# Biblbrox/ViT-Spectre-Experiments

Measured on AMD Instinct MI355X. Metric: images/sec training, Spectre-ViT-S CIFAR-100 bs512, higher is better.
Workload: dtype bf16; 1 GPU; Spectre-ViT-Small (E512 H16 F768 L4 P4 N65, 100 classes, dropout 0.001), fft mixer, train step fwd+CE+bwd+AdamW, bs 512/GPU; mixer=fft, global_batch=512, parallelism=dp1

## Files before the change

include/spv.h:

```cpp
#ifndef SPV_H
#define SPV_H

#include <stddef.h>
#include <stdint.h>

#ifdef __cplusplus
extern "C" {
#endif

#define SPV_F32 0
#define SPV_BF16 1

#define SPV_ABI_VERSION 1

int spv_version(void);
enum {
    SPV_PATH_GEMM_STRIP = 0,
    SPV_PATH_GEMM_STRIP_ACC = 1,
    SPV_PATH_GEMM_TN = 2,
    SPV_PATH_TAIL_LC = 3,
    SPV_PATH_TAIL_UP = 4,
    SPV_PATH_TAIL_LN = 5,
    SPV_PATH_FNET_MFMA = 6,
    SPV_PATH_GATHER_LDS = 7,
// ... 212 lines not shown
#define SPV_HADAMARD_REFUSE_TOKENS (-4)
#define SPV_HADAMARD_REFUSE_WORKSPACE (-5)
int spv_hadamard_path(int dtype, int tokens, int dim, int has_workspace);
int64_t spv_hadamard_workspace_floats(int batch, int tokens, int dim);
int spv_hadamard_mix(const void* x, void* y, const void* add_in, int batch, int tokens, int dim, float scale, int dtype,
                     float* workspace, void* stream);
int spv_hadamard_ln_supported(int tokens, int dim, int dtype);
int spv_hadamard_ln_fwd(const void* x, void* prenorm, void* out, const float* gamma, const float* beta, float* mean, float* rstd,
                        float scale, int batch, int tokens, int dim, int dtype, void* stream);
int spv_hadamard_ln_bwd(const void* dout, const void* prenorm, const float* mean, const float* rstd, const float* gamma, void* dx,
                        float* dgamma, float* dbeta, float* partials, float scale, int batch, int tokens, int dim, int dtype,
                        void* stream);
int spv_hadamard_cls_supported(int tokens, int dim, int dtype);
int spv_hadamard_cls_fwd(const void* x, const float* gamma, const float* beta, void* out, float* m0, float* mean, float* rstd,
                         float scale, int batch, int tokens, int dim, int dtype, void* stream);
int spv_hadamard_cls_bwd(const void* g1, const float* m0, const float* mean, const float* rstd, const float* gamma, void* dx,
                         float* partials, float scale, int batch, int tokens, int dim, int dtype, void* stream);

int spv_patchify(const float* img, void* out, int batch, int chans, int height, int width, int patch, int ld,
                 int transposed, int out_dtype, void* stream);
int spv_patchify_u8(const unsigned char* img_hwc, const float* mean, const float* inv_std, void* out, int batch, int chans,
                    int height, int width, int patch, int ld, int transposed, int out_dtype, void* stream);
int spv_embed_posbias(const float* pos, const float* bias, const float* cls, float* out, int patches, int embed, void* stream);
int spv_embed_cls_rows(const float* cls, const float* pos, void* tokens, int batch, int tokens_per_image, int embed,
                       int dtype, void* stream);
int spv_spectral_fold(const float* proj_w, const float* freq_h, const float* freq_w, float* w_full, int embed,
                      int chans, int patch, void* stream);
int spv_spectral_fold_bf16(const float* proj_w, const float* freq_h, const float* freq_w, float* w_full, void* w_full_bf16, int embed,
                           int chans, int patch, void* stream);
int spv_spectral_fold_bwd(const float* dw_full, const float* proj_w, const float* freq_h, const float* freq_w,
                          float* dproj_w, float* dfreq_h, float* dfreq_w, float* scratch, int embed, int chans,
                          int patch, void* stream);
int spv_dropout(const void* x, void* y, int64_t n, float p, uint64_t seed, int dtype, void* stream);
int spv_embed_bwd_groups(int batch);
int spv_embed_bwd(const void* g, const void* gcls, void* dtok, float* partials, float* dpos, float* dbias, float* dcls, int batch,
                  int tokens, int embed, float p_drop, uint64_t seed, int dtype, void* stream);

int spv_attention_fwd(const void* qkv, void* ctx, void* probs, int seqs, int len, int heads, int head_dim, int dtype,
                      float p_drop, uint64_t seed, void* stream);
int spv_attention_bwd(const void* dctx, const void* qkv, const void* probs, void* dscores, void* dqkv, int seqs, int len,
                      int heads, int head_dim, int dtype, float p_drop, uint64_t seed, void* stream);
int spv_attention_row0_fwd(const void* q0, const void* k, const void* v, int ldkv, void* ctx0, float* probs, int batch, int len,
                           int heads, int head_dim, int dtype, float p_drop, uint64_t seed, void* stream);
int spv_attention_row0_bwd(const void* dctx0, const void* q0, const void* k, const void* v, int ldkv, const float* probs, void* dq0,
                           void* dk, void* dv, int ldd, int batch, int len, int heads, int head_dim, int dtype, float p_drop,
                           uint64_t seed, void* stream);

int spv_gelu_fwd(const void* x, void* y, int64_t n, int dtype, void* stream);
int spv_gelu_bwd(const void* dy, const void* x, void* dx, int64_t n, int dtype, void* stream);
int spv_colsum(const void* x, float* out, float* partials, int rows, int n, int dtype, void* stream);
int spv_axpby(const void* x, const void* y, void* out, float a, float b, int64_t n, int dtype, void* stream);

int spv_small_sl_supported(int rows, int n, int k);
int64_t spv_small_sl_partial_floats(int rows, int n);
int spv_small_sl_fwd(const void* xa, int64_t lda, const void* xb, int64_t ldb, const float* W, const float* bias,
                     const float* gamma, const float* beta, float* out, float* h, float* xs, float* mean, float* rstd,
                     int rows, int n, int k, int dtype, void* stream);
int spv_small_sl_bwd(const float* dout, const float* h, const float* xs, const float* mean, const float* rstd,
                     const float* W, const float* gamma, const float* beta, float* dh, void* dx, float* dW,
                     float* dgamma, float* dbeta, float* dbias, float* partials, int rows, int n, int k, int dx_dtype,
                     void* stream);
int spv_small_sl_bwd_rows(const float* dout, const float* h, const float* mean, const float* rstd, const float* W,
                          const float* gamma, const float* beta, float* dh, void* dx, float* partials, int rows, int n, int k,
                          int dx_dtype, void* stream);
int spv_small_sl_bwd_w(const float* dh, const float* xs, const float* partials, float* dW, float* dgamma, float* dbeta,
                       float* dbias, int rows, int n, int k, void* stream);
// ... 112 lines not shown
```

vit-spectre-experiments_amd/csrc/spv_patch.hip:

```cpp
#define SPV_USES_SEED
#include "spv_common.h"
#include "spv_prologue_core.h"

namespace {

__device__ __forceinline__ float ld_any(const void* base, size_t off, int bf) {
    return bf ? bf2f(static_cast<const bf16_t*>(base)[off]) : static_cast<const float*>(base)[off];
}

__global__ __launch_bounds__(256) void patchify_kernel(const float* __restrict__ img, void* __restrict__ out, int B, int C, int H,
                                                       int W, int P, int ld, int transposed, int bf) {
    patchify_body(img, out, B, C, H, W, P, ld, transposed, bf, blockIdx.x, gridDim.x);
}

template <typename T>
__global__ __launch_bounds__(256) void patchify_vec4_kernel(const float* __restrict__ img, T* __restrict__ out, int B, int C, int H, int W,
                                                            int P, int ld, int token_rows) {
    patchify_vec4_body<T>(img, out, B, C, H, W, P, ld, token_rows, blockIdx.x, gridDim.x);
}

__global__ __launch_bounds__(256) void patchify_u8_kernel(const unsigned char* __restrict__ img, const float* __restrict__ mean,
                                                          const float* __restrict__ inv_std, void* __restrict__ out, int B, int C,
                                                          int H, int W, int P, int ld, int transposed, int bf) {
    const int nH = H / P, nW = W / P, Np = nH * nW, K = C * P * P;
    const int64_t rows = (int64_t)B * Np;
    const int64_t total = transposed == 1 ? (int64_t)K * ld : (transposed == 2 ? (int64_t)B * (Np + 1) * ld : rows * ld);
    for (int64_t e = (int64_t)blockIdx.x * blockDim.x + threadIdx.x; e < total; e += (int64_t)gridDim.x * blockDim.x) {
        int64_t row;
        int k;
        if (transposed == 1) { k = (int)(e / ld); row = e % ld; }
        else { row = e / ld; k = (int)(e % ld); }
        if (transposed == 2) {
            const int64_t b2 = row / (Np + 1);
            const int t2 = (int)(row % (Np + 1));
            row = t2 == 0 ? rows : b2 * Np + t2 - 1;
// ... 77 lines not shown
    }
}
__global__ __launch_bounds__(1024) void freq_weight_grad_kernel(const float* __restrict__ gw, const float* __restrict__ fh,
                                                                const float* __restrict__ fw, float* __restrict__ dfh,
                                                                float* __restrict__ dfw, int EC, int P) {
    extern __shared__ float lds[];
    const int Pv = P / 2 + 1, S = P + Pv;
    const int nt = blockDim.x;
    float* mine = lds + threadIdx.x * S;
    for (int j = 0; j < S; ++j) mine[j] = 0.0f;
    for (int ec = threadIdx.x; ec < EC; ec += nt) {
        const float* g = gw + (size_t)ec * P * Pv;
        for (int u = 0; u < P; ++u)
            for (int v = 0; v < Pv; ++v) {
                const float t = g[u * Pv + v];
                mine[u] += t * fw[v];
                mine[P + v] += t * fh[u];
            }
    }
    for (int stride = nt >> 1; stride >= 1; stride >>= 1) {
        __syncthreads();
        if ((int)threadIdx.x < stride) {
            const float* other = lds + (threadIdx.x + stride) * S;
            for (int j = 0; j < S; ++j) mine[j] += other[j];
        }
    }
    if (threadIdx.x == 0) {
        for (int j = 0; j < P; ++j) dfh[j] = mine[j];
        for (int j = 0; j < Pv; ++j) dfw[j] = mine[P + j];
    }
}

inline int ew_blocks(int64_t n) { return patch_ew_blocks(n); }

}

extern "C" int spv_patchify(const float* img, void* out, int batch, int chans, int height, int width, int patch, int ld,
                            int transposed, int out_dtype, void* stream) {
    SPV_CHECK(batch > 0 && chans > 0 && patch > 0 && height >= patch && width >= patch, "spv_patchify: bad shape");
    SPV_CHECK(out_dtype == SPV_F32 || out_dtype == SPV_BF16, "spv_patchify: bad dtype");
    const int Np = (height / patch) * (width / patch), K = chans * patch * patch;
    const int64_t rows = (int64_t)batch * Np;
    SPV_CHECK(transposed >= 0 && transposed <= 2 && (transposed == 1 ? ld >= rows : ld >= K), "spv_patchify: ld=%d too small", ld);
    const int64_t total = transposed == 1 ? (int64_t)K * ld : (transposed == 2 ? (int64_t)batch * (Np + 1) * ld : rows * ld);
    if (transposed != 1 && patch % 4 == 0 && width % 4 == 0 && ld % 4 == 0 && ((uintptr_t)img & 15) == 0 && ((uintptr_t)out & 15) == 0) {
        const int64_t vecs = (int64_t)batch * (Np + (transposed == 2 ? 1 : 0)) * (ld / 4);
        if (out_dtype == SPV_BF16)
            hipLaunchKernelGGL((patchify_vec4_kernel<bf16_t>), dim3(ew_blocks(vecs)), dim3(256), 0, static_cast<hipStream_t>(stream), img, (bf16_t*)out,
                               batch, chans, height, width, patch, ld, transposed == 2);
        else
            hipLaunchKernelGGL((patchify_vec4_kernel<float>), dim3(ew_blocks(vecs)), dim3(256), 0, static_cast<hipStream_t>(stream), img, (float*)out,
                               batch, chans, height, width, patch, ld, transposed == 2);
        SPV_LAUNCH_CHECK("spv_patchify(vec4)");
        return 0;
    }
    hipLaunchKernelGGL(patchify_kernel, dim3(ew_blocks(total)), dim3(256), 0, static_cast<hipStream_t>(stream), img, out, batch,
                       chans, height, width, patch, ld, transposed, out_dtype == SPV_BF16);
    SPV_LAUNCH_CHECK("spv_patchify");
    return 0;
}

extern "C" int spv_patchify_u8(const unsigned char* img_hwc, const float* mean, const float* inv_std, void* out, int batch,
                               int chans, int height, int width, int patch, int ld, int transposed, int out_dtype, void* stream) {
    SPV_CHECK(batch > 0 && chans > 0 && patch > 0 && height >= patch && width >= patch, "spv_patchify_u8: bad shape");
    SPV_CHECK(out_dtype == SPV_F32 || out_dtype == SPV_BF16, "spv_patchify_u8: bad dtype");
    SPV_CHECK(mean != nullptr && inv_std != nullptr, "spv_patchify_u8: mean / inv_std missing");
    const int Np = (height / patch) * (width / patch), K = chans * patch * patch;
    const int64_t rows = (int64_t)batch * Np;
    SPV_CHECK(transposed >= 0 && transposed <= 2 && (transposed == 1 ? ld >= rows : ld >= K), "spv_patchify_u8: ld=%d too small", ld);
    const int64_t total = transposed == 1 ? (int64_t)K * ld : (transposed == 2 ? (int64_t)batch * (Np + 1) * ld : rows * ld);
    hipLaunchKernelGGL(patchify_u8_kernel, dim3(ew_blocks(total)), dim3(256), 0, static_cast<hipStream_t>(stream), img_hwc, mean,
                       inv_std, out, batch, chans, height, width, patch, ld, transposed, out_dtype == SPV_BF16);
    SPV_LAUNCH_CHECK("spv_patchify_u8");
    return 0;
}

extern "C" int spv_embed_posbias(const float* pos, const float* bias, const float* cls, float* out, int patches, int embed, void* stream) {
    SPV_CHECK(patches > 0 && embed > 0, "spv_embed_posbias: empty");
    hipLaunchKernelGGL(posbias_kernel, dim3(ew_blocks((int64_t)(patches + 1) * embed)), dim3(256), 0, static_cast<hipStream_t>(stream), pos,
                       bias, cls, out, patches, embed);
    SPV_LAUNCH_CHECK("spv_embed_posbias");
    return 0;
}

extern "C" int spv_embed_cls_rows(const float* cls, const float* pos, void* tokens, int batch, int tokens_per_image, int embed,
                                  int dtype, void* stream) {
    SPV_CHECK(batch > 0 && tokens_per_image > 0 && embed > 0, "spv_embed_cls_rows: empty");
    SPV_CHECK(dtype == SPV_F32 || dtype == SPV_BF16, "spv_embed_cls_rows: bad dtype");
    hipLaunchKernelGGL(cls_rows_kernel, dim3(ew_blocks((int64_t)batch * embed)), dim3(256), 0, static_cast<hipStream_t>(stream), cls,
                       pos, tokens, batch, tokens_per_image, embed, dtype == SPV_BF16);
    SPV_LAUNCH_CHECK("spv_embed_cls_rows");
    return 0;
}

constexpr int EB_GS = 16, EB_HB = 8;
template <typename T>
__global__ __launch_bounds__(256) void embed_bwd_rows_kernel(const T* __restrict__ g, const T* __restrict__ gcls, T* __restrict__ dtok,
                                                            float* __restrict__ partials, int B, int TE, int E, float p, uint64_t seed) {
    const int v = blockIdx.x * 256 + threadIdx.x;
    if (v * 8 >= TE) return;
    const int col = v * 8;
    const int b0 = blockIdx.y * EB_GS;
    const float inv_keep = 1.0f / (1.0f - p);
    const uint64_t sd = live_seed(seed);
    float acc[8];
#pragma unroll
    for (int u = 0; u < 8; ++u) acc[u] = 0.0f;
    const bool cls_row = gcls != nullptr && col < E;
    if constexpr (sizeof(T) == 2) {
        typedef unsigned raw4 __attribute__((ext_vector_type(4)));
        for (int h0 = 0; h0 < EB_GS; h0 += EB_HB) {
            raw4 xr[EB_HB], cr[EB_HB];
#pragma unroll
            for (int s = 0; s < EB_HB; ++s) xr[s] = *reinterpret_cast<const raw4*>(g + (size_t)min(b0 + h0 + s, B - 1) * TE + col);
            if (cls_row) {
#pragma unroll
                for (int s = 0; s < EB_HB; ++s) cr[s] = *reinterpret_cast<const raw4*>(gcls + (size_t)min(b0 + h0 + s, B - 1) * E + col);
            }
#pragma unroll
            for (int s = 0; s < EB_HB; ++s) {
                const int b = b0 + h0 + s;
                if (b >= B) break;
                const size_t i = (size_t)b * TE + col;
                float x[8];
// ... 182 lines not shown
```

vit-spectre-experiments_amd/spectre_vit/_native.py:

```python
import ctypes
import os

import torch

_HERE = os.path.dirname(os.path.abspath(__file__))
LIB_PATH = os.environ.get("SPV_LIB_PATH") or os.path.join(os.path.dirname(_HERE), "lib", "libspv_hip.so")

c_vp, c_i, c_i64, c_u64, c_f, c_d = ctypes.c_void_p, ctypes.c_int, ctypes.c_int64, ctypes.c_uint64, ctypes.c_float, ctypes.c_double

PATH = dict(gemm_strip=0, gemm_strip_acc=1, gemm_tn=2, tail_lc=3, tail_up=4, tail_ln=5, fnet_mfma=6, gather_lds=7, distill_cached=8, gemm_tn_wide=9,
            gemm_tn_batch=10, gemm_strip_pool=11, permut_row0=12, gemm_rows=13,
            spectrum=14, conv_fwd=15, conv_dgrad=16, conv_wgrad=17, token_pool=18, token_unpool=19, attn_row0_fwd=20, attn_row0_bwd=21, augment=22, teacher_view=23,
            attn_v1=24, attn_v2=25, attn_v3=26)

SIGNATURES = {
    "spv_version": [],
    "spv_last_error": [],
    "spv_path_count": [c_i],
    "spv_cast": [c_vp, c_i, c_vp, c_i, c_i64, c_vp],
    "spv_cast_transpose": [c_vp, c_i, c_vp, c_i, c_i, c_i, c_i, c_i, c_i, c_i, c_vp],
    "spv_weight_shadows": [c_vp, c_vp, c_vp, c_i, c_i, c_i, c_i, c_vp],
    "spv_weight_shadows_multi": [c_vp, c_vp, c_vp, c_vp, c_i, c_i, c_vp],
    "spv_gemm_nt": [c_vp, c_vp, c_vp, c_vp, c_i, c_i, c_i, c_i, c_i, c_i, c_i, c_i, c_i, c_i, c_vp, c_vp],
    "spv_gemm_nt_grouped_rows": [c_vp, c_vp, c_vp, c_vp, c_vp, c_i, c_i, c_i, c_i, c_i, c_i, c_i, c_i, c_i, c_i, c_i, c_vp],
# ... 29 lines not shown
    "spv_gemm_tn_batch_part": [c_vp, c_i, c_i, c_i, c_vp, c_vp, c_i, c_i, c_vp],
    "spv_small_sl_supported": [c_i, c_i, c_i],
    "spv_small_sl_partial_floats": [c_i, c_i],
    "spv_small_sl_fwd": [c_vp, c_i64, c_vp, c_i64, c_vp, c_vp, c_vp, c_vp, c_vp, c_vp, c_vp, c_vp, c_vp, c_i, c_i, c_i, c_i, c_vp],
    "spv_small_sl_bwd": [c_vp] * 15 + [c_i, c_i, c_i, c_i, c_vp],
    "spv_small_sl_bwd_rows": [c_vp] * 10 + [c_i, c_i, c_i, c_i, c_vp],
    "spv_small_sl_bwd_w": [c_vp] * 7 + [c_i, c_i, c_i, c_vp],
    "spv_cross_entropy_workspace_floats": [],
    "spv_cross_entropy_fwd": [c_vp, c_vp, c_vp, c_vp, c_vp, c_i, c_i, c_vp],
    "spv_cross_entropy_bwd": [c_vp, c_vp, c_vp, c_vp, c_vp, c_i, c_i, c_vp],
    "spv_permut_gather_fwd": [c_vp, c_vp, c_vp, c_vp, c_i, c_i, c_i, c_i, c_i, c_vp],
    "spv_gemm_nt_pool_bwd": [c_vp, c_vp, c_vp, c_vp, c_i, c_i, c_i, c_i, c_i, c_i, c_i, c_i, c_i, c_i, c_vp],
    "spv_permut_gather_bwd": [c_vp, c_vp, c_vp, c_i, c_i, c_i, c_i, c_vp],
    "spv_fnet_mix": [c_vp, c_vp, c_vp, c_vp, c_i, c_i, c_i, c_i, c_vp, c_vp],
    "spv_fnet_workspace_floats": [c_i, c_i, c_i],
    "spv_fnet_twiddle_floats": [c_i],
    "spv_fnet_make_twiddle": [c_vp, c_i, c_vp],
    "spv_fnet_ln_supported": [c_i, c_i, c_i],
    "spv_fnet_cls_supported": [c_i, c_i, c_i],
    "spv_fnet_cls_fwd": [c_vp, c_vp, c_vp, c_vp, c_vp, c_vp, c_vp, c_i, c_i, c_i, c_i, c_vp],
    "spv_fnet_cls_bwd": [c_vp, c_vp, c_vp, c_vp, c_vp, c_vp, c_vp, c_i, c_i, c_i, c_i, c_vp],
    "spv_fnet_ln_fwd": [c_vp, c_vp, c_vp, c_vp, c_vp, c_vp, c_vp, c_vp, c_i, c_i, c_i, c_i, c_vp],
    "spv_fnet_ln_bwd": [c_vp, c_vp, c_vp, c_vp, c_vp, c_vp, c_vp, c_vp, c_vp, c_vp, c_i, c_i, c_i, c_i, c_vp],
    "spv_rfft_real": [c_vp, c_vp, c_i, c_i, c_i, c_i, c_vp],
    "spv_haar_dwt": [c_vp, c_vp, c_i, c_i, c_i, c_i, c_i, c_i, c_i, c_vp, c_vp],
    "spv_patchify": [c_vp, c_vp, c_i, c_i, c_i, c_i, c_i, c_i, c_i, c_i, c_vp],
    "spv_patchify_u8": [c_vp, c_vp, c_vp, c_vp, c_i, c_i, c_i, c_i, c_i, c_i, c_i, c_i, c_vp],
    "spv_embed_posbias": [c_vp, c_vp, c_vp, c_vp, c_i, c_i, c_vp],
    "spv_embed_cls_rows": [c_vp, c_vp, c_vp, c_i, c_i, c_i, c_i, c_vp],
    "spv_spectral_fold": [c_vp, c_vp, c_vp, c_vp, c_i, c_i, c_i, c_vp],
    "spv_spectral_fold_bf16": [c_vp, c_vp, c_vp, c_vp, c_vp, c_i, c_i, c_i, c_vp],
    "spv_spectral_fold_bwd": [c_vp, c_vp, c_vp, c_vp, c_vp, c_vp, c_vp, c_vp, c_i, c_i, c_i, c_vp],
    "spv_dropout": [c_vp, c_vp, c_i64, c_f, c_u64, c_i, c_vp],
    "spv_attention_fwd": [c_vp, c_vp, c_vp, c_i, c_i, c_i, c_i, c_i, c_f, c_u64, c_vp],
    "spv_attention_bwd": [c_vp, c_vp, c_vp, c_vp, c_vp, c_i, c_i, c_i, c_i, c_i, c_f, c_u64, c_vp],
    "spv_attention_row0_fwd": [c_vp, c_vp, c_vp, c_i, c_vp, c_vp, c_i, c_i, c_i, c_i, c_i, c_f, c_u64, c_vp],
    "spv_attention_row0_bwd": [c_vp, c_vp, c_vp, c_vp, c_i, c_vp, c_vp, c_vp, c_vp, c_i, c_i, c_i, c_i, c_i, c_i, c_f, c_u64, c_vp],
    "spv_gelu_fwd": [c_vp, c_vp, c_i64, c_i, c_vp],
    "spv_gelu_bwd": [c_vp, c_vp, c_vp, c_i64, c_i, c_vp],
    "spv_colsum": [c_vp, c_vp, c_vp, c_i, c_i, c_i, c_vp],
    "spv_set_seed_device_ptr": [c_vp],
    "spv_seed_advance": [c_vp, c_vp],
    "spv_step_prologue": [c_vp, c_vp],
    "spv_adamw_multi": [c_vp, c_vp, c_vp, c_vp, c_i, c_f, c_f, c_f, c_f, c_f, c_f, c_f, c_f, c_f, c_vp, c_vp],
    "spv_adamw_multi_ema": [c_vp, c_vp, c_vp, c_vp, c_i, c_f, c_f, c_f, c_f, c_f, c_f, c_f, c_f, c_f, c_vp, c_vp, c_f, c_i, c_f, c_vp],
    "spv_grad_sumsq": [c_vp, c_vp, c_vp, c_vp, c_i, c_vp, c_vp],
    "spv_step_control": [c_vp, c_i, c_vp, c_i, c_vp, c_i, c_i, c_i, c_d, c_f, c_vp],
    "spv_adamw_multi_ctl": [c_vp, c_vp, c_vp, c_vp, c_i, c_d, c_f, c_f, c_f, c_f, c_f, c_f, c_vp, c_vp, c_vp],
    "spv_adamw_multi_ctl_ema": [c_vp, c_vp, c_vp, c_vp, c_i, c_d, c_f, c_f, c_f, c_f, c_f, c_f, c_vp, c_vp, c_vp, c_f, c_i, c_vp],
    "spv_fwht": [c_vp, c_vp, c_vp, c_i, c_i, c_i, c_i, c_i, c_i, c_f, c_i, c_vp],
    "spv_hadamard_path": [c_i, c_i, c_i, c_i],
    "spv_hadamard_workspace_floats": [c_i, c_i, c_i],
    "spv_hadamard_mix": [c_vp, c_vp, c_vp, c_i, c_i, c_i, c_f, c_i, c_vp, c_vp],
    "spv_hadamard_ln_supported": [c_i, c_i, c_i],
    "spv_hadamard_ln_fwd": [c_vp, c_vp, c_vp, c_vp, c_vp, c_vp, c_vp, c_f, c_i, c_i, c_i, c_i, c_vp],
    "spv_hadamard_ln_bwd": [c_vp, c_vp, c_vp, c_vp, c_vp, c_vp, c_vp, c_vp, c_vp, c_f, c_i, c_i, c_i, c_i, c_vp],
    "spv_hadamard_cls_supported": [c_i, c_i, c_i],
    "spv_hadamard_cls_fwd": [c_vp, c_vp, c_vp, c_vp, c_vp, c_vp, c_vp, c_f, c_i, c_i, c_i, c_i, c_vp],
    "spv_hadamard_cls_bwd": [c_vp, c_vp, c_vp, c_vp, c_vp, c_vp, c_vp, c_f, c_i, c_i, c_i, c_i, c_vp],
    "spv_axpby":[c_vp, c_vp, c_vp, c_f, c_f, c_i64, c_i, c_vp],
    "spv_spectrum_floats": [c_i, c_i],
    "spv_spectrum_log1p": [c_vp, c_vp, c_i, c_i, c_i, c_i, c_i, c_vp],
    "spv_conv3x3_fwd": [c_vp, c_vp, c_vp, c_vp, c_vp, c_i, c_i, c_i, c_i, c_i, c_i, c_vp],
    "spv_conv3x3_dgrad": [c_vp, c_vp, c_vp, c_vp, c_i, c_i, c_i, c_i, c_i, c_i, c_vp],
    "spv_conv3x3_wgrad": [c_vp, c_vp, c_vp, c_vp, c_vp, c_vp, c_i, c_i, c_i, c_i, c_i, c_i, c_i, c_vp],
    "spv_token_pool_fwd": [c_vp, c_vp, c_i, c_i, c_i, c_i, c_i, c_i, c_vp],
# ... 3 lines not shown
    "spv_augment_u8": [c_vp, c_vp, c_vp, c_vp, c_vp, c_vp, c_i, c_i, c_i, c_i, c_i, c_vp],
    "spv_augment_plan": [c_i, c_i, c_i],
    "spv_augment_tiled_ws_bytes": [c_i, c_i, c_i],
    "spv_augment_tiled_u8": [c_vp, c_vp, c_vp, c_vp, c_vp, c_vp, c_i, c_i, c_i, c_i, c_i, c_vp, ctypes.c_size_t, c_vp],
    "spv_teacher_view_supported": [c_i, c_i, c_i, c_i],
    "spv_teacher_view_u8": [c_vp, c_vp, c_vp, c_vp, c_vp, c_i, c_i, c_i, c_i, c_i, c_i, c_i, c_vp],
    "spv_distill_loss_workspace_floats": [],
    "spv_distill_loss_fwd": [c_vp, c_vp, c_vp, c_vp, c_vp, c_vp, c_i, c_i, c_f, c_f, c_f, c_vp],
    "spv_distill_loss_bwd": [c_vp, c_vp, c_vp, c_vp, c_vp, c_vp, c_i, c_i, c_f, c_f, c_f, c_vp],
    "spv_logit_cache_store": [c_vp, c_vp, c_vp, c_i, c_i, c_i, c_vp],
    "spv_distill_loss_idx_fwd": [c_vp, c_vp, c_vp, c_vp, c_vp, c_vp, c_vp, c_i, c_i, c_i, c_f, c_f, c_f, c_vp],
    "spv_distill_loss_idx_bwd": [c_vp, c_vp, c_vp, c_vp, c_vp, c_vp, c_vp, c_i, c_i, c_i, c_f, c_f, c_f, c_vp],
    "spv_eval_head_stats_words": [],
    "spv_eval_head": [c_vp, c_vp, c_vp, c_vp, c_vp, c_i, c_i, c_i, c_i, c_vp],
    "spv_train_meter_words": [c_i64],
    "spv_cross_entropy_meter_workspace_floats": [],
    "spv_cross_entropy_meter_fwd": [c_vp, c_vp, c_vp, c_vp, c_vp, c_i, c_i, c_vp, c_i, c_vp],
    "spv_distill_loss_meter_workspace_floats": [],
    "spv_distill_loss_meter_fwd": [c_vp, c_vp, c_vp, c_vp, c_vp, c_vp, c_i, c_i, c_f, c_f, c_f, c_vp, c_i, c_vp],
    "spv_distill_loss_idx_meter_fwd": [c_vp, c_vp, c_vp, c_vp, c_vp, c_vp, c_vp, c_i, c_i, c_i, c_f, c_f, c_f, c_vp, c_i, c_vp],
    "spv_loader_cursor_bytes": [],
    "spv_loader_fetch": [c_vp] * 8 + [c_i] * 8 + [c_u64, c_i, c_i, c_i, c_vp],
    "spv_loader_augment_supported": [c_i, c_i, c_i],
    "spv_loader_fetch_augment": [c_vp] * 10 + [c_i] * 8 + [c_u64, c_i, c_i, c_u64, c_vp],
    "spv_loader_augment_tiled_supported": [c_i, c_i, c_i],
    "spv_loader_fetch_augment_tiled": [c_vp] * 10 + [c_i] * 8 + [c_u64, c_i, c_i, c_u64, c_vp, ctypes.c_size_t, c_vp],
}
_RESTYPES = {"spv_last_error": ctypes.c_char_p, "spv_path_count": ctypes.c_longlong, "spv_rowop_partial_floats": c_i64, "spv_fnet_workspace_floats": c_i64,
             "spv_fnet_twiddle_floats": c_i64, "spv_tail_ln_partial_floats": c_i64, "spv_permut_table_words": c_i64, "spv_small_sl_partial_floats": c_i64,
             "spv_cross_entropy_workspace_floats": c_i64, "spv_distill_loss_workspace_floats": c_i64,
             "spv_eval_head_stats_words": c_i64, "spv_augment_tiled_ws_bytes": ctypes.c_size_t, "spv_train_meter_words": c_i64,
             "spv_cross_entropy_meter_workspace_floats": c_i64, "spv_distill_loss_meter_workspace_floats": c_i64,
             "spv_loader_cursor_bytes": c_i64, "spv_hadamard_workspace_floats": c_i64}
_NO_STATUS = set(_RESTYPES) | {"spv_hadamard_path", "spv_hadamard_ln_supported", "spv_hadamard_cls_supported", "spv_version", "spv_fnet_ln_supported", "spv_fnet_cls_supported", "spv_tail_ln_supported", "spv_tail_up_supported", "spv_small_sl_supported", "spv_tail_bwd_parts", "spv_embed_bwd_groups", "spv_haar_ln_supported", "spv_permut_pool_supported", "spv_spectrum_floats", "spv_augment_supported", "spv_loader_augment_supported", "spv_loader_augment_tiled_supported", "spv_augment_plan", "spv_teacher_view_supported"}

class FoldJob(ctypes.Structure):
    _fields_ = [("partials", c_vp), ("out", c_vp * 5), ("parts", c_i), ("nsum", c_i), ("n", c_i)]


class AugmentCfg(ctypes.Structure):
    _fields_ = [(n, c_f) for n in ("flip_p", "bright_lo", "bright_hi", "contrast_lo", "contrast_hi", "sat_lo", "sat_hi", "hue_lo", "hue_hi",
                                   "gray_p", "degrees", "blur_p", "sigma_lo", "sigma_hi", "erase_p", "scale_lo", "scale_hi", "ratio_lo",
                                   "ratio_hi")]


class PrologueJobs(ctypes.Structure):
    _fields_ = ([("seed_word", c_vp), ("shadow_table", c_vp), ("tile_tensor", c_vp), ("tile_x", c_vp), ("tile_y", c_vp), ("ntiles", c_i),
                 ("shadow_dtype", c_i), ("fold_w", c_vp), ("fold_fh", c_vp), ("fold_fw", c_vp), ("fold_out", c_vp), ("fold_out_bf16", c_vp)]
                + [(n, c_i) for n in ("fold_embed", "fold_chans", "fold_patch", "pad0")]
                + [("patch_img", c_vp), ("patch_out", c_vp)]
                + [(n, c_i) for n in ("patch_batch", "patch_chans", "patch_height", "patch_width", "patch_size", "patch_ld", "patch_dtype", "pad1")]
                + [("pos_pos", c_vp), ("pos_bias", c_vp), ("pos_cls", c_vp), ("pos_out", c_vp), ("pos_patches", c_i), ("pos_embed", c_i)])


class TnProblem(ctypes.Structure):
    _fields_ = [("a", c_vp), ("b", c_vp), ("c", c_vp), ("m", c_i), ("n", c_i), ("lda", c_i), ("ldb", c_i), ("ldc", c_i), ("k", c_i)]


_lib = None
timer = None
hint = 0
_LAUNCHERS = {}


def load():
    global _lib
    if _lib is None:
# ... 36 lines not shown
```

vit-spectre-experiments_amd/spectre_vit/hip_ops.py:

```python
from __future__ import annotations

import collections
import ctypes
import os
import warnings
import weakref
from typing import NamedTuple

import torch

from . import _native, prologue, shadows
from ._launch import _DT, BF16, F32, _dt, _p, _require_gpu, _stream
from .shadows import invalidate_weight_shadows
from .timing import KernelTimer, _timing, set_kernel_timer


_warned_fp16 = False


def compute_dtype(x: torch.Tensor) -> torch.dtype:
    global _warned_fp16
    if torch.is_autocast_enabled("cuda"):
        dt = torch.get_autocast_dtype("cuda")
        if dt == torch.float16:
# ... 709 lines not shown
        _require_gpu(img, w_full)
        u8 = img.dtype == torch.uint8
        if u8:
            if norm is None:
                raise ValueError("uint8 images need the (mean, inv_std) normalisation tensors")
            B, H, W, C = img.shape
        else:
            B, C, H, W = img.shape
        E, K = w_full.shape
        Np = (H // patch) * (W // patch)
        T = Np + 1
        dev = img.device
        img = img.contiguous() if u8 else img.contiguous().float()
        _check_channels("patch embedding", E, K, dtype)
        st = _stream()
        patches = None if u8 else prologue.take("patchify", (img,), (patch, dtype))
        if patches is not None:
            pass
        elif u8:
            patches = torch.empty((B * T, K), dtype=dtype, device=dev)
            _native.call("spv_patchify_u8", _p(img), _p(norm[0]), _p(norm[1]), _p(patches), B, C, H, W, patch, K, 2, _DT[dtype], st)
        else:
            patches = torch.empty((B * T, K), dtype=dtype, device=dev)
            _native.call("spv_patchify", _p(img), _p(patches), B, C, H, W, patch, K, 2, _DT[dtype], st)
        wc = w_full if dtype == torch.float32 else (getattr(w_full, "_spv_bf16", None) if dtype == torch.bfloat16 else None)
        if wc is None:
            wc = _raw_cast(w_full, dtype)
        posbias = prologue.take("posbias", (pos, bias, cls), (Np, E))
        if posbias is None:
            posbias = torch.empty((T, E), dtype=torch.float32, device=dev)
            _native.call("spv_embed_posbias", _p(pos), _p(bias), _p(cls), _p(posbias), Np, E, st)
        tokens = torch.empty((B, T, E), dtype=dtype, device=dev)
        seed = _new_seed() if p_drop > 0.0 else 0
        _native.call("spv_gemm_nt_grouped_rows_drop", _p(patches), _p(wc), 0, _p(posbias), _p(tokens), B * T, E, K, K, K, E,
                     _DT[dtype], _DT[dtype], T, T, 0, float(p_drop), seed, st)
        ctx.save_for_backward(None if u8 else img, patches if (dtype == torch.bfloat16 or u8) else None)
        ctx.meta = (B, C, H, W, patch, E, K, Np, T, dtype, cls.shape, pos.shape, float(p_drop), seed)
        ctx.sinks = (_sink(bias), _sink(cls), _sink(pos))
        ctx.key = _EmbedKey()
        tokens._spv_embed_key = ctx.key
        return tokens

    @staticmethod
    def backward(ctx, dtok):
        img, patches = ctx.saved_tensors
        B, C, H, W, patch, E, K, Np, T, dtype, cls_shape, pos_shape, p_drop, seed = ctx.meta
        dev = dtok.device
        st = _stream()
        dtok = dtok.contiguous()
        early = start_held_wgrads()
        gcls = _cls_grad_stash.pop(ctx.key, None)
        if gcls is not None:
            gcls = gcls.to(dtok.dtype).contiguous()
        s_bias, s_cls, s_pos = ctx.sinks
        dpos_full = _grad_buf(s_pos, pos_shape, dev)
        dbias = _grad_buf(s_bias, (E,), dev)
        dcls = _grad_buf(s_cls, cls_shape, dev)
        part = torch.empty((_native.call("spv_embed_bwd_groups", B) * T * E,), dtype=torch.float32, device=dev)
        masked = torch.empty_like(dtok) if (gcls is not None or p_drop > 0.0) else None
        _native.call("spv_embed_bwd", _p(dtok), _p(gcls), _p(masked), _p(part), _p(dpos_full), _p(dbias), _p(dcls), B, T, E, p_drop, seed,
                     _dt(dtok), st)
        if masked is not None:
            dtok = masked
        if patches is not None and dtok.dtype == torch.bfloat16:
            dwf = _weight_grad(dtok.view(B * T, E), patches, B * T, E, K)
            flush_held_head()
            if not early:
                join_side_stream()
# ... 154 lines not shown
        _native.call("spv_permut_row0_bwd", _p(dg0), _p(dx0), _p(ctx.table), _p(dx), B, N * E, n, E, _DT[dtype], _stream())
        return dx, None, None


def _cls_row_gradient(shape, dtype, dev, rows):
    if shape[1] == 1:
        return rows.to(dtype).reshape(shape)
    key = (tuple(shape), dtype, dev.index)
    full = _cls_grad_bufs.get(key)
    if full is None:
        if len(_cls_grad_bufs) > 8:
            _cls_grad_bufs.clear()
        full = torch.zeros(shape, dtype=dtype, device=dev)
        _cls_grad_bufs[key] = full
    full[:, 0, :] = rows
    return full


class ClsAddFn(torch.autograd.Function):

    @staticmethod
    def forward(ctx, out, src_cls):
        _require_gpu(out, src_cls)
        ctx.meta = (out.shape, out.dtype)
        return out[:, 0, :] + src_cls

    @staticmethod
    def backward(ctx, g):
        shape, dtype = ctx.meta
        return _cls_row_gradient(shape, dtype, g.device, g), g


STEP_PROLOGUE = True


def step_prologue(model, img, seed_word, autocast_dtype):
    prologue.clear()
    if not STEP_PROLOGUE:
        _native.call("spv_seed_advance", _p(seed_word), _stream())
        return
    jobs = _native.PrologueJobs()
    jobs.seed_word = _p(seed_word)
    work = 16.0
    deposits = []
    emb = getattr(model, "embeddings_block", None)
    if autocast_dtype == torch.bfloat16 and torch.is_grad_enabled() and img.is_cuda:
        weights_fn = getattr(model, "_shadow_weights", None)
        weights = weights_fn() if callable(weights_fn) else None
        ss = shadows.shadow_set(model, weights) if weights else None
        if ss is not None and ss.dtype == torch.bfloat16:
            table, tt, tx, ty, ntiles = ss._tables
            jobs.shadow_table, jobs.tile_tensor, jobs.tile_x, jobs.tile_y = _p(table), _p(tt), _p(tx), _p(ty)
            jobs.ntiles, jobs.shadow_dtype = ntiles, BF16
            work += 2048.0 * ntiles * 8
            deposits.append(("shadows", weights, (ss.dtype,), ss))
        sources_fn = getattr(emb, "_prologue_sources", None)
        sources = sources_fn(img) if callable(sources_fn) and img.dtype == torch.float32 and img.is_contiguous() else None
        if sources is not None:
            (w, fh, fw, C, P), (bias, cls, pos) = sources
            B, _, H, W = img.shape
            dev = img.device
            E, K = w.shape[0], C * P * P
            Np = (H // P) * (W // P)
            fp32 = all(t.dtype == torch.float32 and t.is_contiguous() and t.is_cuda for t in (w, fh, fw, pos, bias, cls))
            if fp32 and P > 0 and H >= P and W >= P and w.dim() == 2 and w.shape[1] == C * P * (P // 2 + 1) and pos.numel() == (Np + 1) * E:
                wf = torch.empty((E, K), dtype=torch.float32, device=dev)
# ... 851 lines not shown
```

vit-spectre-experiments_amd/spectre_vit/timing.py:

```python
from __future__ import annotations

import torch

from . import _native
from ._launch import BF16, F32

PEAK_TFLOPS = {BF16: 2500.0, F32: 157.3}
PEAK_HBM_GBS = 8000.0


def _es(dt):
    return 2 if dt == BF16 else 4


_WORK_MODELS = {
    "spv_small_sl_fwd": lambda i: ("head_fwd", i[2:5], i[5], "mfma", 2.0 * i[2] * i[3] * i[4]),
    "spv_small_sl_bwd": lambda i: ("head_bwd", i[0:3], i[3], "mfma", 4.0 * i[0] * i[1] * i[2]),
    "spv_small_sl_bwd_rows": lambda i: ("head_bwd_rows", i[0:3], i[3], "mfma", 2.0 * i[0] * i[1] * i[2]),
    "spv_small_sl_bwd_w": lambda i: ("head_bwd_w", i[0:3], F32, "mfma", 2.0 * i[0] * i[1] * i[2]),
    "spv_cross_entropy_fwd": lambda i: ("cross_entropy_fwd", i[0:2], F32, "hbm", i[0] * i[1] * 4.0),
    "spv_cross_entropy_bwd": lambda i: ("cross_entropy_bwd", i[0:2], F32, "hbm", i[0] * i[1] * 8.0),
    "spv_distill_loss_fwd": lambda i: ("distill_loss_fwd", i[0:2], F32, "hbm", i[0] * i[1] * 8.0),
    "spv_distill_loss_bwd": lambda i: ("distill_loss_bwd", i[0:2], F32, "hbm", i[0] * i[1] * 12.0),
    "spv_distill_loss_idx_fwd": lambda i: ("distill_loss_idx_fwd", (i[0], i[2]), F32, "hbm", i[0] * (i[2] * 8.0 + 8.0)),
    "spv_distill_loss_idx_bwd": lambda i: ("distill_loss_idx_bwd", (i[0], i[2]), F32, "hbm", i[0] * (i[2] * 12.0 + 8.0)),
    "spv_cross_entropy_meter_fwd": lambda i: ("cross_entropy_meter_fwd", i[0:2], F32, "hbm", i[0] * i[1] * 4.0),
    "spv_distill_loss_meter_fwd": lambda i: ("distill_loss_meter_fwd", i[0:2], F32, "hbm", i[0] * i[1] * 8.0),
    "spv_distill_loss_idx_meter_fwd": lambda i: ("distill_loss_idx_meter_fwd", (i[0], i[2]), F32, "hbm", i[0] * (i[2] * 8.0 + 8.0)),
    "spv_logit_cache_store": lambda i: ("logit_cache_store", (i[0], i[2]), F32, "hbm", i[0] * (i[2] * 8.0 + 8.0)),
    "spv_teacher_view_u8": lambda i: ("teacher_view", (i[0], i[2], i[3], i[5]), i[6], "hbm",
                                      1.0 * i[0] * i[2] * (i[3] * i[3] + i[5] * i[5] * _es(i[6]))),
    "spv_gemm_nt": lambda i: ("gemm_acc" if i[8] else "gemm", i[0:3], i[6], "mfma", 2.0 * i[0] * i[1] * i[2]),
    "spv_gemm_nt_grouped_rows": lambda i: ("gemm_grouped_rows", i[0:3], i[6], "mfma", 2.0 * i[0] * i[1] * i[2]),
    "spv_gemm_nt_grouped_rows_drop": lambda i: ("gemm_grouped_rows", i[0:3], i[6], "mfma", 2.0 * i[0] * i[1] * i[2]),
    "spv_gemm_nt_pool_bwd": lambda i: ("gemm_pool_bwd", i[1:4], i[7], "mfma", 2.0 * i[1] * i[2] * i[3]),
    "spv_gemm_tn": lambda i: ("gemm_tn", i[0:3], BF16, "mfma", 2.0 * i[0] * i[1] * i[2]),
    "spv_gemm_tn_fold": lambda i: ("gemm_tn", i[0:3], BF16, "mfma", 2.0 * i[0] * i[1] * i[2]),
    "spv_gemm_tn_batch_part": lambda i: (("gemm_tn_batch", i[0:3], BF16, "mfma", float(i[-1])) if i[4] == 1 else
                                         ("splitk_reduce_batch", i[0:4], F32, "hbm", float(i[-1]))),
    "spv_embed_bwd": lambda i: ("embed_bwd", i[0:3], i[3], "hbm", 1.0 * i[0] * i[1] * i[2] * _es(i[3]) * (1 if (i[-2] >> 2) & 1 else 2)),
    "spv_fnet_cls_fwd": lambda i: ("fnet_cls_fwd", i[0:3], i[3], "hbm", 1.0 * i[0] * (i[1] + 1) * i[2] * _es(i[3])),
    "spv_fnet_cls_bwd": lambda i: ("fnet_cls_bwd", i[0:3], i[3], "hbm", 1.0 * i[0] * (i[1] + 1) * i[2] * _es(i[3])),
    "spv_permut_row0_fwd": lambda i: ("permut_row0_fwd", i[0:4], i[4], "hbm", 2.0 * i[0] * (i[2] + i[3]) * _es(i[4])),
    "spv_permut_row0_bwd": lambda i: ("permut_row0_bwd", i[0:4], i[4], "hbm", 1.0 * i[0] * (i[1] + i[2] + i[3]) * _es(i[4])),
    "spv_patchify": lambda i: ("patchify", i[0:5], i[7], "hbm",
                               1.0 * i[0] * i[1] * i[2] * i[3] * 4 + 1.0 * i[0] * ((i[2] // i[4]) * (i[3] // i[4]) + (i[6] == 2)) * i[5] * _es(i[7])),
    "spv_weight_shadows_multi": lambda i: ("weight_shadows_multi", i[0:1], i[1], "hbm", 2048.0 * i[0] * (4 + 2 * _es(i[1]))),
    "spv_spectre_tail_fwd": lambda i: ("tail_fwd", i[0:3], i[3], "hbm", i[0] * (2.0 * i[1] + i[2]) * _es(i[3])),
    "spv_spectre_tail_bwd": lambda i: ("tail_bwd" if not (i[-2] >> 7) & 1 else "tail_bwd_nodx", i[0:3], i[3], "hbm",
                                       i[0] * (3.0 * i[1] + (0 if (i[-2] >> 7) & 1 else i[2])) * _es(i[3])),
    "spv_spectre_tail_bwd_up": lambda i: ("tail_bwd_up", i[0:3], i[3], "hbm", i[0] * (3.0 * i[1] + 3.0 * i[2]) * _es(i[3])),
    "spv_spectre_tail_ln_fwd": lambda i: ("tail_ln_fwd", i[0:3], i[3], "hbm", i[0] * (4.0 * i[1] + i[2]) * _es(i[3])),
    "spv_spectre_tail_ln_bwd": lambda i: ("tail_ln_bwd", i[0:3], i[3], "hbm", i[0] * 6.0 * i[1] * _es(i[3])),
    "spv_add_layernorm_fwd": lambda i: ("addln_fwd", i[0:2], i[3], "hbm", 3.0 * i[0] * i[1] * _es(i[3])),
    "spv_add_layernorm_bwd": lambda i: ("addln_bwd", i[0:2], i[3], "hbm", (3.0 + (i[2] == 1)) * i[0] * i[1] * _es(i[3])),
    "spv_permut_gather_fwd": lambda i: ("gather_fwd", i[1:4], i[4], "hbm", i[1] * i[3] * (1.0 + i[2]) * _es(i[4])),
    "spv_permut_gather_bwd": lambda i: ("gather_bwd", i[0:3], i[3], "hbm", i[0] * i[2] * (1.0 + i[1]) * _es(i[3])),
    "spv_fnet_mix": lambda i: ("fnet_mix", i[0:3], i[3], "hbm", 2.0 * i[0] * i[1] * i[2] * _es(i[3])),
    "spv_fnet_ln_fwd": lambda i: ("fnet_ln_fwd", i[0:3], i[3], "hbm", 3.0 * i[0] * i[1] * i[2] * _es(i[3])),
    "spv_fnet_ln_bwd": lambda i: ("fnet_ln_bwd", i[0:3], i[3], "hbm", 3.0 * i[0] * i[1] * i[2] * _es(i[3])),
    "spv_haar_ln_fwd": lambda i: ("haar_ln_fwd", i[0:2], i[2], "hbm", 2.0 * i[0] * i[1] * _es(i[2])),
    "spv_haar_ln_bwd": lambda i: ("haar_ln_bwd", i[0:2], i[2], "hbm", 3.0 * i[0] * i[1] * _es(i[2])),
    "spv_haar_dwt": lambda i: ("haar_dwt", i[0:3], i[6], "hbm", 2.0 * i[0] * i[1] * i[2] * _es(i[6])),
    "spv_adamw_multi": lambda i: ("adamw_multi", i[0:1], F32, "hbm", 7.0 * 4 * 2048 * i[0]),
    "spv_adamw_multi_ema": lambda i: ("adamw_multi_ema", i[0:1], F32, "hbm", 9.0 * 4 * 2048 * i[0]),
    "spv_adamw_multi_ctl_ema": lambda i: ("adamw_multi_ctl_ema", i[0:1], F32, "hbm", 9.0 * 4 * 2048 * i[0]),
    "spv_grad_sumsq": lambda i: ("grad_sumsq", i[0:1], F32, "hbm", 4.0 * 2048 * i[0]),
# ... 90 lines not shown
```

Measured before the change: 318,800 images/sec.

## Add persistent MFMA token-embed kernel with fused posbias and dropout

```diff
diff --git a/include/spv.h b/include/spv.h
--- a/include/spv.h
+++ b/include/spv.h
@@ -268,6 +268,9 @@
                           float* dproj_w, float* dfreq_h, float* dfreq_w, float* scratch, int embed, int chans,
                           int patch, void* stream);
 int spv_dropout(const void* x, void* y, int64_t n, float p, uint64_t seed, int dtype, void* stream);
+int spv_token_embed_supported(int rows, int n, int k, int dtype);
+int spv_token_embed_fwd(const void* patches, const void* w, const float* posbias, void* tokens, int rows, int n, int k,
+                        int tokens_per_image, float p_drop, uint64_t seed, void* stream);
 int spv_embed_bwd_groups(int batch);
 int spv_embed_bwd(const void* g, const void* gcls, void* dtok, float* partials, float* dpos, float* dbias, float* dcls, int batch,
                   int tokens, int embed, float p_drop, uint64_t seed, int dtype, void* stream);
diff --git a/vit-spectre-experiments_amd/csrc/spv_patch.hip b/vit-spectre-experiments_amd/csrc/spv_patch.hip
--- a/vit-spectre-experiments_amd/csrc/spv_patch.hip
+++ b/vit-spectre-experiments_amd/csrc/spv_patch.hip
@@ -1,6 +1,9 @@
 #define SPV_USES_SEED
 #include "spv_common.h"
 #include "spv_prologue_core.h"
+#include "spv_token_embed_core.h"
+
+#include <type_traits>
 
 namespace {
 
@@ -144,6 +147,114 @@
 }
 
 inline int ew_blocks(int64_t n) { return patch_ew_blocks(n); }
+
+template <int KS>
+__global__ __launch_bounds__(64 * TE_WAVES, 3) void token_embed_kernel(const bf16_t* __restrict__ P, const bf16_t* __restrict__ Wt,
+                                                                    const float* __restrict__ posbias, bf16_t* __restrict__ out, int rows,
+                                                                    int n, int T, int shares, int walkers, float p, uint64_t seed) {
+    constexpr int K = 16 * KS;
+    constexpr int SLD = TE_COLS + 4;
+    __shared__ __attribute__((aligned(16))) float stage_all[TE_WAVES][16 * SLD];
+    const int lane = threadIdx.x & 63, wave = threadIdx.x >> 6;
+    const int g = blockIdx.x * TE_WAVES + wave;
+    if (g >= shares * walkers) return;
+    const int walker = g / shares, n0 = (g % shares) * TE_COLS;
+    const int frow = lane & 31, fh = lane >> 5;
+    float* st = stage_all[wave];
+
+    uint4 b[2][KS];
+#pragma unroll
+    for (int j = 0; j < 2; ++j)
+#pragma unroll
+        for (int s = 0; s < KS; ++s) b[j][s] = *reinterpret_cast<const uint4*>(Wt + (size_t)(n0 + 32 * j + frow) * K + 16 * s + 8 * fh);
+    const uint64_t seed_live = p > 0.0f ? live_seed(seed) : 0;
+    const float inv_keep = 1.0f / (1.0f - p);
+    const int nblk = (rows + TE_ROWS - 1) / TE_ROWS;
+    const int lr0 = lane >> 3, c8 = lane & 7;
+    const int col0 = n0 + c8 * 8;
+
+    auto load_a = [&](int rb, uint4 (&a)[KS]) {
+        const bf16_t* ap = P + (size_t)min(rb * TE_ROWS + frow, rows - 1) * K + 8 * fh;
+#pragma unroll
+        for (int s = 0; s < KS; ++s) a[s] = *reinterpret_cast<const uint4*>(ap + 16 * s);
+    };
+    const int step8 = 8 % T, stepw = (int)(((int64_t)walkers * TE_ROWS) % T);
+    auto wrap = [&](int t) { return t - (t >= T ? T : 0); };
+    float4 pb[4][2];
+    auto load_pb = [&](int q, int t) {
+        const float* pp = posbias + (size_t)t * n + col0;
+        pb[q][0] = *reinterpret_cast<const float4*>(pp);
+        pb[q][1] = *reinterpret_cast<const float4*>(pp + 4);
+    };
+    uint4 a[KS];
+    load_a(walker, a);
+    int t0 = (walker * TE_ROWS + lr0) % T;
+    {
+        int t = t0;
+#pragma unroll
+        for (int q = 0; q < 4; ++q) { load_pb(q, t); t = wrap(t + step8); }
+    }
+    auto block = [&](int rb, auto masked_tag) __attribute__((always_inline)) {
+        constexpr bool MASKED = decltype(masked_tag)::value;
+        f32x16 acc[2];
+#pragma unroll
+        for (int j = 0; j < 2; ++j)
+#pragma unroll
+            for (int r = 0; r < 16; ++r) acc[j][r] = 0.0f;
+#pragma unroll
+        for (int s = 0; s < KS; ++s)
+#pragma unroll
+            for (int j = 0; j < 2; ++j)
+                acc[j] = __builtin_amdgcn_mfma_f32_32x32x16_bf16(__builtin_bit_cast(bf16x8, a[s]), __builtin_bit_cast(bf16x8, b[j][s]), acc[j], 0, 0, 0);
+        load_a(min(rb + walkers, nblk - 1), a);
+        t0 = wrap(t0 + stepw);
+        {
+            uint4 o[4];
+            int tn = t0;
+#pragma unroll
+            for (int h = 0; h < 2; ++h) {
+#pragma unroll
+                for (int j = 0; j < 2; ++j)
+#pragma unroll
+                    for (int r = 0; r < 8; ++r) st[((r & 3) + 8 * (r >> 2) + 4 * fh) * SLD + 32 * j + frow] = acc[j][8 * h + r];
+                __builtin_amdgcn_fence(__ATOMIC_RELEASE, "wavefront");
+#pragma unroll
+                for (int t = 0; t < 2; ++t) {
+                    const int q = 2 * h + t, lr = lr0 + 8 * t;
+                    const float4 lo = *reinterpret_cast<const float4*>(st + lr * SLD + c8 * 8);
+                    const float4 hi = *reinterpret_cast<const float4*>(st + lr * SLD + c8 * 8 + 4);
+                    float v[8] = {lo.x, lo.y, lo.z, lo.w, hi.x, hi.y, hi.z, hi.w};
+                    const float4 p0 = pb[q][0], p1 = pb[q][1];
+                    v[0] += p0.x; v[1] += p0.y; v[2] += p0.z; v[3] += p0.w; v[4] += p1.x; v[5] += p1.y; v[6] += p1.z; v[7] += p1.w;
+                    load_pb(q, tn);
+                    tn = wrap(tn + step8);
+                    if (p > 0.0f) {
+                        const size_t fi = (size_t)(rb * TE_ROWS + lr0 + 8 * q) * n + col0;
+                        const unsigned key = dropout_row_key(seed_live, (uint64_t)(unsigned)(fi >> 12));
+                        const unsigned key_base = key + ((unsigned)(fi & 4095) >> 1) * 0x9e3779b1u;
+#pragma unroll
+                        for (int u = 0; u < 8; ++u) v[u] *= dropout_scale_at(key_base, u, p, inv_keep);
+                    }
+                    o[q].x = pack_bf16x2(v[0], v[1]);
+                    o[q].y = pack_bf16x2(v[2], v[3]);
+                    o[q].z = pack_bf16x2(v[4], v[5]);
+                    o[q].w = pack_bf16x2(v[6], v[7]);
+                }
+                __builtin_amdgcn_fence(__ATOMIC_RELEASE, "wavefront");
+            }
+            __builtin_amdgcn_sched_barrier(0);
+#pragma unroll
+            for (int q = 0; q < 4; ++q) {
+                const int row = rb * TE_ROWS + lr0 + 8 * q;
+                if (!MASKED || row < rows) *reinterpret_cast<uint4*>(out + (size_t)row * n + col0) = o[q];
+            }
+        }
+    };
+    const int nfull = rows / TE_ROWS;
+    int rb = walker;
+    for (; rb < nfull; rb += walkers) block(rb, std::false_type{});
+    if (rb < nblk) block(rb, std::true_type{});
+}
 
 }
 
@@ -202,6 +313,41 @@
     hipLaunchKernelGGL(cls_rows_kernel, dim3(ew_blocks((int64_t)batch * embed)), dim3(256), 0, static_cast<hipStream_t>(stream), cls,
                        pos, tokens, batch, tokens_per_image, embed, dtype == SPV_BF16);
     SPV_LAUNCH_CHECK("spv_embed_cls_rows");
+    return 0;
+}
+
+extern "C" int spv_token_embed_supported(int rows, int n, int k, int dtype) { return token_embed_supported(rows, n, k, dtype); }
+
+extern "C" int spv_token_embed_fwd(const void* patches, const void* w, const float* posbias, void* tokens, int rows, int n, int k,
+                                   int tokens_per_image, float p_drop, uint64_t seed, void* stream) {
+    SPV_CHECK(token_embed_supported(rows, n, k, SPV_BF16) && (int64_t)rows * n <= (1ll << 40),
+              "spv_token_embed_fwd: unsupported shape %d x %d x %d (bf16; k a multiple of 16 in 16..64; n a multiple of 64; rows * n <= 2^40)", rows, n, k);
+    SPV_CHECK(tokens_per_image > 0, "spv_token_embed_fwd: tokens_per_image=%d", tokens_per_image);
+    SPV_CHECK(p_drop >= 0.0f && p_drop < 1.0f, "spv_token_embed_fwd: p_drop=%f", p_drop);
+    SPV_CHECK(patches && w && posbias && tokens, "spv_token_embed_fwd: null pointer");
+    SPV_CHECK((((uintptr_t)patches | (uintptr_t)w | (uintptr_t)posbias | (uintptr_t)tokens) & 15) == 0,
+              "spv_token_embed_fwd: pointers must be 16-byte aligned");
+    static int cus = 0;
+    if (cus == 0) {
+        int dev = 0, v = 0;
+        SPV_CHECK(hipGetDevice(&dev) == hipSuccess && hipDeviceGetAttribute(&v, hipDeviceAttributeMultiprocessorCount, dev) == hipSuccess && v > 0,
+                  "spv_token_embed_fwd: no device to size the grid for");
+        cus = v;
+    }
+    const TokenEmbedPlan pl = token_embed_plan(rows, n, cus);
+    hipStream_t st = static_cast<hipStream_t>(stream);
+#define SPV_TOKEN_EMBED(KS)                                                                                                      \
+    hipLaunchKernelGGL((token_embed_kernel<KS>), dim3(pl.grid), dim3(64 * TE_WAVES), 0, st, static_cast<const bf16_t*>(patches), \
+                       static_cast<const bf16_t*>(w), posbias, static_cast<bf16_t*>(tokens), rows, n, tokens_per_image, pl.shares, \
+                       pl.walkers, p_drop, seed)
+    switch (k / 16) {
+    case 1: SPV_TOKEN_EMBED(1); break;
+    case 2: SPV_TOKEN_EMBED(2); break;
+    case 3: SPV_TOKEN_EMBED(3); break;
+    default: SPV_TOKEN_EMBED(4); break;
+    }
+#undef SPV_TOKEN_EMBED
+    SPV_LAUNCH_CHECK("spv_token_embed_fwd");
     return 0;
 }
 
diff --git a/vit-spectre-experiments_amd/csrc/spv_token_embed_core.h b/vit-spectre-experiments_amd/csrc/spv_token_embed_core.h
--- /dev/null
+++ b/vit-spectre-experiments_amd/csrc/spv_token_embed_core.h
@@ -0,0 +1,26 @@
+#pragma once
+#include <stdint.h>
+
+constexpr int TE_ROWS = 32, TE_COLS = 64;
+constexpr int TE_WAVES = 4;
+constexpr int TE_WAVES_PER_CU = 12;
+constexpr int TE_DT_BF16 = 1;
+
+inline int token_embed_supported(int rows, int n, int k, int dtype) {
+    return dtype == TE_DT_BF16 && rows > 0 && n > 0 && n % TE_COLS == 0 && k >= 16 && k <= 64 && k % 16 == 0;
+}
+
+struct TokenEmbedPlan {
+    int shares, walkers, per, grid;
+};
+inline TokenEmbedPlan token_embed_plan(int rows, int n, int cus) {
+    TokenEmbedPlan p{};
+    p.shares = n / TE_COLS;
+    const int nblk = (int)(((int64_t)rows + TE_ROWS - 1) / TE_ROWS);
+    int most = (int)((int64_t)cus * TE_WAVES_PER_CU / p.shares);
+    if (most < 1) most = 1;
+    p.per = (nblk + most - 1) / most;
+    p.walkers = (nblk + p.per - 1) / p.per;
+    p.grid = (int)(((int64_t)p.walkers * p.shares + TE_WAVES - 1) / TE_WAVES);
+    return p;
+}
diff --git a/vit-spectre-experiments_amd/spectre_vit/_native.py b/vit-spectre-experiments_amd/spectre_vit/_native.py
--- a/vit-spectre-experiments_amd/spectre_vit/_native.py
+++ b/vit-spectre-experiments_amd/spectre_vit/_native.py
@@ -85,6 +85,8 @@
     "spv_spectral_fold_bf16": [c_vp, c_vp, c_vp, c_vp, c_vp, c_i, c_i, c_i, c_vp],
     "spv_spectral_fold_bwd": [c_vp, c_vp, c_vp, c_vp, c_vp, c_vp, c_vp, c_vp, c_i, c_i, c_i, c_vp],
     "spv_dropout": [c_vp, c_vp, c_i64, c_f, c_u64, c_i, c_vp],
+    "spv_token_embed_supported": [c_i, c_i, c_i, c_i],
+    "spv_token_embed_fwd": [c_vp, c_vp, c_vp, c_vp, c_i, c_i, c_i, c_i, c_f, c_u64, c_vp],
     "spv_attention_fwd": [c_vp, c_vp, c_vp, c_i, c_i, c_i, c_i, c_i, c_f, c_u64, c_vp],
     "spv_attention_bwd": [c_vp, c_vp, c_vp, c_vp, c_vp, c_i, c_i, c_i, c_i, c_i, c_f, c_u64, c_vp],
     "spv_attention_row0_fwd": [c_vp, c_vp, c_vp, c_i, c_vp, c_vp, c_i, c_i, c_i, c_i, c_i, c_f, c_u64, c_vp],
@@ -154,7 +156,7 @@
              "spv_eval_head_stats_words": c_i64, "spv_augment_tiled_ws_bytes": ctypes.c_size_t, "spv_train_meter_words": c_i64,
              "spv_cross_entropy_meter_workspace_floats": c_i64, "spv_distill_loss_meter_workspace_floats": c_i64,
              "spv_loader_cursor_bytes": c_i64, "spv_hadamard_workspace_floats": c_i64}
-_NO_STATUS = set(_RESTYPES) | {"spv_hadamard_path", "spv_hadamard_ln_supported", "spv_hadamard_cls_supported", "spv_version", "spv_fnet_ln_supported", "spv_fnet_cls_supported", "spv_tail_ln_supported", "spv_tail_up_supported", "spv_small_sl_supported", "spv_tail_bwd_parts", "spv_embed_bwd_groups", "spv_haar_ln_supported", "spv_permut_pool_supported", "spv_spectrum_floats", "spv_augment_supported", "spv_loader_augment_supported", "spv_loader_augment_tiled_supported", "spv_augment_plan", "spv_teacher_view_supported"}
+_NO_STATUS = set(_RESTYPES) | {"spv_hadamard_path", "spv_hadamard_ln_supported", "spv_hadamard_cls_supported", "spv_version", "spv_fnet_ln_supported", "spv_fnet_cls_supported", "spv_tail_ln_supported", "spv_tail_up_supported", "spv_small_sl_supported", "spv_tail_bwd_parts", "spv_embed_bwd_groups", "spv_haar_ln_supported", "spv_permut_pool_supported", "spv_spectrum_floats", "spv_augment_supported", "spv_loader_augment_supported", "spv_loader_augment_tiled_supported", "spv_augment_plan", "spv_teacher_view_supported", "spv_token_embed_supported"}
 
 class FoldJob(ctypes.Structure):
     _fields_ = [("partials", c_vp), ("out", c_vp * 5), ("parts", c_i), ("nsum", c_i), ("n", c_i)]
diff --git a/vit-spectre-experiments_amd/spectre_vit/hip_ops.py b/vit-spectre-experiments_amd/spectre_vit/hip_ops.py
--- a/vit-spectre-experiments_amd/spectre_vit/hip_ops.py
+++ b/vit-spectre-experiments_amd/spectre_vit/hip_ops.py
@@ -765,8 +765,12 @@
             _native.call("spv_embed_posbias", _p(pos), _p(bias), _p(cls), _p(posbias), Np, E, st)
         tokens = torch.empty((B, T, E), dtype=dtype, device=dev)
         seed = _new_seed() if p_drop > 0.0 else 0
-        _native.call("spv_gemm_nt_grouped_rows_drop", _p(patches), _p(wc), 0, _p(posbias), _p(tokens), B * T, E, K, K, K, E,
-                     _DT[dtype], _DT[dtype], T, T, 0, float(p_drop), seed, st)
+        if TOKEN_EMBED_KERNEL and _native.call("spv_token_embed_supported", B * T, E, K, _DT[dtype]):
+            _native.call("spv_token_embed_fwd", _p(patches), _p(wc), _p(posbias), _p(tokens), B * T, E, K, T, float(p_drop), seed, st)
+            PATH_COUNTS["token_embed"] += 1
+        else:
+            _native.call("spv_gemm_nt_grouped_rows_drop", _p(patches), _p(wc), 0, _p(posbias), _p(tokens), B * T, E, K, K, K, E,
+                         _DT[dtype], _DT[dtype], T, T, 0, float(p_drop), seed, st)
         ctx.save_for_backward(None if u8 else img, patches if (dtype == torch.bfloat16 or u8) else None)
         ctx.meta = (B, C, H, W, patch, E, K, Np, T, dtype, cls.shape, pos.shape, float(p_drop), seed)
         ctx.sinks = (_sink(bias), _sink(cls), _sink(pos))
@@ -987,6 +991,7 @@
 
 
 STEP_PROLOGUE = True
+TOKEN_EMBED_KERNEL = True
 
 
 def step_prologue(model, img, seed_word, autocast_dtype):
diff --git a/vit-spectre-experiments_amd/spectre_vit/timing.py b/vit-spectre-experiments_amd/spectre_vit/timing.py
--- a/vit-spectre-experiments_amd/spectre_vit/timing.py
+++ b/vit-spectre-experiments_amd/spectre_vit/timing.py
@@ -33,6 +33,7 @@
     "spv_gemm_nt": lambda i: ("gemm_acc" if i[8] else "gemm", i[0:3], i[6], "mfma", 2.0 * i[0] * i[1] * i[2]),
     "spv_gemm_nt_grouped_rows": lambda i: ("gemm_grouped_rows", i[0:3], i[6], "mfma", 2.0 * i[0] * i[1] * i[2]),
     "spv_gemm_nt_grouped_rows_drop": lambda i: ("gemm_grouped_rows", i[0:3], i[6], "mfma", 2.0 * i[0] * i[1] * i[2]),
+    "spv_token_embed_fwd": lambda i: ("gemm_grouped_rows", i[0:3], BF16, "mfma", 2.0 * i[0] * i[1] * i[2]),
     "spv_gemm_nt_pool_bwd": lambda i: ("gemm_pool_bwd", i[1:4], i[7], "mfma", 2.0 * i[1] * i[2] * i[3]),
     "spv_gemm_tn": lambda i: ("gemm_tn", i[0:3], BF16, "mfma", 2.0 * i[0] * i[1] * i[2]),
     "spv_gemm_tn_fold": lambda i: ("gemm_tn", i[0:3], BF16, "mfma", 2.0 * i[0] * i[1] * i[2]),
```

Result: faster. 322,100 images/sec (median of 6 runs) (+1.0%).
